# ctxnn/GenConViT

Hardware: AMD Instinct MI355X
Metric: frames/sec (224x224, ed+vae forward) (higher is better)
Workload: dtype f16

## Files before the change

### genconvit_amd/_lib.py

```python
from __future__ import annotations

import ctypes
import ctypes.util
import json
import os
import threading

_HERE = os.path.dirname(os.path.abspath(__file__))
LIB_PATH = os.environ.get("GCV_LIB_PATH") or os.path.join(_HERE, "lib", "libgenconvit_hip.so")

GCV_F32, GCV_BF16, GCV_F16 = 0, 1, 2
ACT_NONE, ACT_RELU, ACT_GELU, ACT_LEAKY = 0, 1, 2, 3
A_PLAIN, A_IM2COL3_POOL, A_IM2COL3_S2 = 0, 1, 2
EPI_BIAS_ACT, EPI_RESID, EPI_POOL4, EPI_CONVT, EPI_SPLITK = 0, 1, 2, 3, 4

c_void_p, c_int, c_int64, c_float, c_char_p, c_size_t = (ctypes.c_void_p, ctypes.c_int, ctypes.c_int64,
                                                         ctypes.c_float, ctypes.c_char_p, ctypes.c_size_t)


class TensorDesc(ctypes.Structure):
    _fields_ = [("name", c_char_p), ("data", c_void_p), ("numel", c_int64), ("on_device", c_int)]


class GemmArgs(ctypes.Structure):
# ... 7 lines not shown
    "gcv_last_error": (c_char_p, []),
    "gcv_create": (c_int, [ctypes.POINTER(c_void_p), c_int, c_int, c_int]),
    "gcv_create_arch": (c_int, [ctypes.POINTER(c_void_p), c_int, c_int, c_int, c_int]),
    "gcv_handle_arch": (c_int, [c_void_p]),
    "gcv_destroy": (None, [c_void_p]),
    "gcv_workspace_bytes": (c_size_t, [c_void_p]),
    "gcv_load_ed": (c_int, [c_void_p, ctypes.POINTER(TensorDesc), c_int]),
    "gcv_load_vae": (c_int, [c_void_p, ctypes.POINTER(TensorDesc), c_int]),
    "gcv_load_swin": (c_int, [c_void_p, ctypes.POINTER(TensorDesc), c_int, c_char_p]),
    "gcv_ed_forward": (c_int, [c_void_p, c_void_p, c_int, c_void_p, c_void_p]),
    "gcv_vae_forward": (c_int, [c_void_p, c_void_p, c_void_p, c_int, c_void_p, c_void_p, c_void_p, c_void_p, c_void_p]),
    "gcv_genconvit_forward": (c_int, [c_void_p, c_void_p, c_void_p, c_void_p, c_int, c_void_p, c_void_p]),
    "gcv_ed_explain": (c_int, [c_void_p, c_void_p, c_int, c_void_p, c_void_p, c_void_p, c_void_p, c_void_p]),
    "gcv_vae_explain": (c_int, [c_void_p, c_void_p, c_void_p, c_int, c_void_p, c_void_p, c_void_p, c_void_p, c_void_p]),
    "gcv_genconvit_explain": (c_int, [c_void_p, c_void_p, c_void_p, c_void_p, c_int, c_void_p, c_void_p, c_void_p,
                                      c_void_p, c_void_p]),
    "gcv_ed_explain_at": (c_int, [c_void_p, c_void_p, c_int, c_void_p, c_int, c_void_p, c_void_p, c_void_p, c_void_p]),
    "gcv_vae_explain_at": (c_int, [c_void_p, c_void_p, c_void_p, c_int, c_void_p, c_int, c_void_p, c_void_p, c_void_p,
                                   c_void_p]),
    "gcv_genconvit_explain_at": (c_int, [c_void_p, c_void_p, c_void_p, c_void_p, c_int, c_void_p, c_int, c_void_p, c_void_p,
                                         c_void_p, c_void_p]),
    "gcv_comm_available": (c_int, []),
    "gcv_comm_count": (c_int, [c_void_p]),
    "gcv_comm_unique_id": (c_int, [c_void_p]),
    "gcv_comm_create": (c_int, [ctypes.POINTER(c_void_p), c_int, c_int, c_void_p, c_int]),
    "gcv_comm_destroy": (None, [c_void_p]),
    "gcv_allgather_logits": (c_int, [c_void_p, c_void_p, c_int, c_void_p, c_void_p]),
    "gcv_convnext_forward": (c_int, [c_void_p, c_int, c_void_p, c_int, c_int, c_void_p, c_void_p]),
    "gcv_swin_forward": (c_int, [c_void_p, c_void_p, c_int, c_void_p, c_void_p]),
    "gcv_vote": (c_int, [c_void_p, c_int, c_void_p, c_void_p]),
    "gcv_preprocess": (c_int, [c_int, c_void_p, c_void_p, c_int, c_int, c_int, c_void_p]),
    "gcv_face_crop_resize": (c_int, [c_void_p, c_int, c_int, c_int, c_void_p, c_int, c_void_p, c_int, c_void_p]),
    "gcv_face_crop_preprocess": (c_int, [c_int, c_void_p, c_int, c_int, c_int, c_void_p, c_int, c_void_p, c_int, c_void_p]),
    "gcv_cam_overlay": (c_int, [c_void_p, c_int, c_int, c_int, c_void_p, c_int, c_void_p, c_int, c_int, c_void_p, c_float,
                                c_int, c_void_p, c_void_p]),
    "gcv_track_match": (c_int, [c_void_p, c_int, c_int, c_int, c_void_p, c_int, c_int, c_int, c_void_p, c_void_p]),
    "gcv_track_chain": (c_int, [c_void_p, c_int, c_int, c_int, c_void_p, c_int, c_int, c_int, c_int, c_void_p, c_void_p]),
    "gcv_frame_hist": (c_int, [c_void_p, c_int, c_int, c_int, c_int, c_void_p, c_void_p]),
    "gcv_hist_diff": (c_int, [c_void_p, c_int, c_int, c_void_p, c_void_p]),
    "gcv_frame_cells": (c_int, [c_void_p, c_int, c_int, c_int, c_int, c_void_p, c_void_p]),
    "gcv_blend_fit": (c_int, [c_void_p, c_int, c_int, c_int, c_void_p, c_void_p]),
    "gcv_hist_diff_lag": (c_int, [c_void_p, c_int, c_int, c_int, c_void_p, c_void_p]),
    "gcv_face_quality": (c_int, [c_void_p, c_int, c_int, c_int, c_void_p, c_int, c_int, c_void_p, c_void_p]),
    "gcv_face_signature": (c_int, [c_void_p, c_int, c_int, c_int, c_void_p, c_int, c_void_p, c_void_p]),
    "gcv_sig_link": (c_int, [c_void_p, c_void_p, c_int, c_int, c_void_p, c_void_p]),
    "gcv_vote_segments": (c_int, [c_void_p, c_int, c_int, c_void_p, c_int, c_void_p, c_void_p]),
    "gcv_vote_windows": (c_int, [c_void_p, c_int, c_int, c_void_p, c_int, c_void_p, c_void_p, c_void_p]),
    "gcv_tap_set": (c_int, [c_void_p, c_char_p, c_void_p, c_size_t]),
    "gcv_tap_clear": (c_int, [c_void_p]),
    "gcv_tap_written": (c_int, [c_void_p, c_char_p]),
    "gcv_profile_enable": (c_int, [c_void_p, c_int]),
    "gcv_profile_report": (c_char_p, [c_void_p]),
    "gcv_k_gemm": (c_int, [c_int, c_int, c_int, ctypes.POINTER(GemmArgs), c_void_p]),
    "gcv_k_stem_ln": (c_int, [c_int, c_void_p, c_int64, c_int64, c_int64, c_int64, c_void_p, c_void_p, c_void_p,
                              c_void_p, c_void_p, c_int, c_int, c_int, c_float, c_void_p]),
    "gcv_k_stem_ln_c": (c_int, [c_int, c_void_p, c_int64, c_int64, c_int64, c_int64, c_void_p, c_void_p, c_void_p,
                                c_void_p, c_void_p, c_int, c_int, c_int, c_int, c_float, c_void_p]),
    "gcv_k_dwconv7_ln": (c_int, [c_int, c_void_p, c_void_p, c_void_p, c_void_p, c_void_p, c_void_p, c_int, c_int,
                                 c_int, c_int, c_float, c_void_p]),
    "gcv_dw_plan": (c_int, [c_int, c_int, c_int, c_int, c_int, c_int, c_void_p]),
    "gcv_convnext_res_ok": (c_int, [c_int, c_int]),
    "gcv_k_ln_patchify": (c_int, [c_int, c_void_p, c_void_p, c_void_p, c_void_p, c_int, c_int, c_int, c_int, c_float,
                                  c_void_p]),
    "gcv_k_layernorm_rows": (c_int, [c_int, c_void_p, c_void_p, c_void_p, c_void_p, c_int64, c_int, c_float, c_void_p]),
    "gcv_k_pool_ln": (c_int, [c_int, c_void_p, c_void_p, c_void_p, c_void_p, c_int, c_int, c_int, c_float, c_void_p]),
    "gcv_k_pool_ln_rows": (c_int, [c_int, c_void_p, c_void_p, c_void_p, c_void_p, c_int, c_int, c_int, c_float, c_int, c_int,
                                   c_int, c_void_p]),
    "gcv_k_conv3_first": (c_int, [c_int, c_void_p, c_int64, c_int64, c_int64, c_int64, c_void_p, c_void_p, c_void_p,
                                  c_int, c_int, c_int, c_int, c_int, c_void_p]),
    "gcv_k_convt2_small": (c_int, [c_int, c_void_p, c_void_p, c_void_p, c_void_p, c_int, c_int, c_int, c_int, c_void_p]),
    "gcv_k_reparam": (c_int, [c_int, c_void_p, c_int, c_void_p, c_void_p, c_void_p, c_void_p, c_int, c_int, c_void_p]),
    "gcv_k_head_tail": (c_int, [c_int, c_void_p, c_void_p, c_void_p, c_void_p, c_int, c_int, c_void_p]),
    "gcv_k_head_tail_splitk": (c_int, [c_int, c_void_p, c_int, c_void_p, c_int, c_void_p, c_void_p, c_void_p, c_int, c_int,
                                       c_void_p]),
    "gcv_k_resize_mse": (c_int, [c_int, c_void_p, c_void_p, c_void_p, c_void_p, c_void_p, c_int, c_void_p]),
    "gcv_k_swin_window_attn": (c_int, [c_int, c_void_p, c_void_p, c_void_p, c_int, c_int, c_int, c_int, c_int, c_int,
                                       c_void_p]),
    "gcv_k_patch_merge_ln": (c_int, [c_int, c_void_p, c_void_p, c_void_p, c_void_p, c_int, c_int, c_int, c_int, c_float,
                                     c_void_p]),
    "gcv_k_mean_tokens": (c_int, [c_int, c_void_p, c_void_p, c_int, c_int, c_int, c_void_p]),
    "gcv_k_head_bwd": (c_int, [c_int, c_void_p, c_int, c_void_p, c_void_p, c_void_p, c_void_p, c_void_p, c_void_p, c_void_p,
                               c_int, c_int, c_void_p]),
    "gcv_k_bb_bwd": (c_int, [c_int, c_void_p, c_void_p, c_void_p, c_int, c_int, c_void_p]),
    "gcv_k_cam": (c_int, [c_int, c_int, c_int, c_void_p, c_void_p, c_int, c_int, c_int, c_int, c_int, c_int, c_void_p,
                          c_void_p, c_void_p, c_void_p, c_float, c_int, c_void_p]),
    "gcv_k_pool_ln_bwd": (c_int, [c_int, c_int, c_int, c_void_p, c_void_p, c_int, c_int, c_int, c_int, c_void_p, c_void_p,
                                  c_void_p, c_float, c_int, c_void_p]),
    "gcv_k_scale_rows": (c_int, [c_int, c_void_p, c_void_p, c_void_p, c_void_p, c_int, c_int, c_void_p]),
    "gcv_k_gelu_bwd": (c_int, [c_int, c_void_p, c_void_p, c_void_p, c_void_p, c_int, c_int, c_void_p]),
    "gcv_k_dw_ln_bwd": (c_int, [c_int, c_void_p, c_void_p, c_void_p, c_void_p, c_void_p, c_void_p, c_void_p, c_int, c_int,
                                c_int, c_float, c_void_p]),
    "gcv_k_dw_dgrad_res": (c_int, [c_void_p, c_void_p, c_void_p, c_int, c_int, c_int, c_void_p]),
    "gcv_k_down_ln_bwd": (c_int, [c_int, c_void_p, c_void_p, c_void_p, c_void_p, c_void_p, c_int, c_int, c_int, c_float,
                                  c_void_p]),
    "gcv_k_cam2": (c_int, [c_int, c_int, c_int, c_void_p, c_void_p, c_void_p, c_void_p, c_int, c_int, c_int, c_int, c_int,
                           c_int, c_void_p, c_void_p, c_void_p, c_int, c_void_p]),
    "gcv_k_fused_mlp": (c_int, [c_int, c_int, c_void_p, c_void_p, c_void_p, c_void_p, c_void_p, c_void_p, c_void_p,
                                c_void_p, c_int, c_void_p]),
    "gcv_k_fused_mlp_lnp": (c_int, [c_int, c_int, c_void_p, c_void_p, c_void_p, c_void_p, c_void_p, c_void_p, c_void_p,
                                    c_void_p, c_void_p, c_float, c_int, c_void_p, c_void_p, c_void_p, c_void_p, c_void_p,
                                    c_int, c_void_p]),
    "gcv_k_fused_mlp_timed": (c_int, [c_int, c_int, c_void_p, c_void_p, c_void_p, c_void_p, c_void_p, c_void_p,
                                      c_void_p, c_void_p, c_int, c_int, c_void_p, c_void_p]),
}

_lib = None
# ... 791 lines not shown
```

### genconvit_amd/csrc/api.hip

```cpp
#include "../../include/genconvit_hip.h"

#include <dlfcn.h>

#include <cstdio>
#include <cstdlib>
#include <cstring>
#include <map>
#include <mutex>
#include <set>
#include <sstream>
#include <vector>

#include "cam.h"
#include "cam_bwd.h"
#include "cnx_mlp.h"
#include "gemm.h"
#include "kernels.h"
#include "net.h"

namespace gcv {
static thread_local std::string g_err;
void set_error(const std::string& msg) { g_err = msg; }
const char* get_error() { return g_err.c_str(); }

int ensure_dynamic_lds(const void* fn, int bytes) {
  static std::mutex mu;
  static std::map<std::pair<const void*, int>, int> done;
  int dev = 0;
  GCV_CHECK_HIP(hipGetDevice(&dev));
  std::lock_guard<std::mutex> lk(mu);
  auto it = done.find({fn, dev});
  if (it != done.end() && it->second >= bytes) return 0;
  GCV_CHECK_HIP(hipFuncSetAttribute(fn, hipFuncAttributeMaxDynamicSharedMemorySize, bytes));
  done[{fn, dev}] = bytes;
  return 0;
}

hipEvent_t Profiler::get_event() {
  if (next_event == pool.size()) {
    hipEvent_t e;
    if (hipEventCreate(&e) != hipSuccess) return nullptr;
    pool.push_back(e);
  }
  return pool[next_event++];
}
Profiler::~Profiler() {
  for (hipEvent_t e : pool) (void)hipEventDestroy(e);
}

namespace {
struct Roctx {
  int (*push)(const char*) = nullptr;
  int (*pop)() = nullptr;
  Roctx() {
    for (const char* lib : {"librocprofiler-sdk-roctx.so", "librocprofiler-sdk-roctx.so.1", "libroctx64.so", "libroctx64.so.4"}) {
      void* h = dlopen(lib, RTLD_NOW | RTLD_GLOBAL);
      if (!h) continue;
      push = reinterpret_cast<int (*)(const char*)>(dlsym(h, "roctxRangePushA"));
      pop = reinterpret_cast<int (*)()>(dlsym(h, "roctxRangePop"));
      if (push && pop) return;
      push = nullptr; pop = nullptr;
    }
  }
};
Roctx& roctx() { static Roctx r; return r; }
}
bool tap_name_known(const std::string& name, int arch) {
  auto make = [](int arch) {
    std::set<std::string> n;
// ... 471 lines not shown
int gcv_tap_written(gcv_handle* h, const char* name) {
  GCV_REQUIRE(h && name, "null handle / tap name");
  auto it = h->net->taps.find(name);
  GCV_REQUIRE(it != h->net->taps.end(), std::string("no tap '") + name + "' is set");
  return it->second.need != 0 && it->second.mask == it->second.need ? 1 : 0;
}

size_t gcv_workspace_bytes(const gcv_handle* h) { return h ? h->net->workspace_bytes() : 0; }

int gcv_handle_arch(const gcv_handle* h) { return h ? h->net->arch : -1; }

int gcv_profile_enable(gcv_handle* h, int on) {
  GCV_REQUIRE(h, "null handle");
  h->net->prof.enabled = on != 0;
  h->net->prof.reset();
  return 0;
}

const char* gcv_profile_report(gcv_handle* h) {
  if (!h) return "[]";
  Profiler& p = h->net->prof;
  struct Agg { int n = 0; double ms = 0, flops = 0, bytes = 0; };
  std::map<std::string, Agg> agg;
  std::vector<std::string> order;
  for (auto& r : p.recs) {
    float ms = 0.0f;
    if (hipEventSynchronize(r.e1) != hipSuccess || hipEventElapsedTime(&ms, r.e0, r.e1) != hipSuccess) ms = -1.0f;
    if (!agg.count(r.tag)) order.push_back(r.tag);
    Agg& a = agg[r.tag];
    a.n += 1; a.ms += ms; a.flops += r.flops; a.bytes += r.bytes;
  }
  std::ostringstream os;
  os.precision(9);
  os << "[";
  for (size_t i = 0; i < order.size(); ++i) {
    const Agg& a = agg[order[i]];
    os << (i ? "," : "") << "{\"tag\":\"" << order[i] << "\",\"launches\":" << a.n << ",\"ms\":" << a.ms
       << ",\"flops\":" << a.flops << ",\"bytes\":" << a.bytes << "}";
  }
  os << "]";
  h->report = os.str();
  p.reset();
  return h->report.c_str();
}

#define DISPATCH_DT(dt, CALL)                                    \
  switch (dt) {                                                  \
    case GCV_F32:  { typedef float T;  return CALL; }            \
    case GCV_BF16: { typedef bf16_t T; return CALL; }            \
    case GCV_F16:  { typedef half_t T; return CALL; }            \
    default: set_error("bad dtype"); return -2;                  \
  }

int gcv_k_gemm(int dtype, int a_mode, int epi, const gcv_gemm_args* a, gcv_stream stream) {
  GCV_REQUIRE(a, "null args");
  GemmArgs g{};
  g.A = a->A; g.Wt = a->Wt; g.C = a->C; g.bias = a->bias; g.gamma = a->gamma; g.resid = a->resid;
  g.partial = a->partial; g.M = a->M; g.N = a->N; g.K = a->K; g.lda = a->lda; g.ldc = a->ldc; g.act = a->act;
  g.splitk = a->splitk; g.k_per_split = a->k_per_split; g.H = a->H; g.W = a->W; g.cin_log2 = a->cin_log2;
  g.cout_log2 = a->cout_log2;
  DISPATCH_DT(dtype, launch_gemm<T>(g, a_mode, epi, (hipStream_t)stream));
}

int gcv_k_stem_ln(int dtype, const void* x, int64_t sb, int64_t sc, int64_t sy, int64_t sx, const float* wp,
                  const float* bias, const float* lnw, const float* lnb, void* out, int nimg, int Ho, int Wo,
                  float eps, gcv_stream s) {
  DISPATCH_DT(dtype, launch_stem_ln<T>((const T*)x, sb, sc, sy, sx, wp, bias, lnw, lnb, (T*)out, nimg, Ho, Wo, eps,
                                       (hipStream_t)s));
}

int gcv_k_stem_ln_c(int dtype, const void* x, int64_t sb, int64_t sc, int64_t sy, int64_t sx, const float* wp,
                    const float* bias, const float* lnw, const float* lnb, void* out, int nimg, int Ho, int Wo, int C,
                    float eps, gcv_stream s) {
  DISPATCH_DT(dtype, launch_stem_ln<T>((const T*)x, sb, sc, sy, sx, wp, bias, lnw, lnb, (T*)out, nimg, Ho, Wo, eps,
                                       (hipStream_t)s, C));
}

int gcv_k_dwconv7_ln(int dtype, const void* x, const float* wdw, const float* bdw, const float* lnw,
                     const float* lnb, void* y, int nimg, int H, int W, int C, float eps, gcv_stream s) {
  DISPATCH_DT(dtype, launch_dwconv7_ln<T>((const T*)x, wdw, bdw, lnw, lnb, (T*)y, nimg, H, W, C, eps, (hipStream_t)s));
}

int gcv_dw_plan(int dtype, int nimg, int H, int W, int C, int aligned, int* out5) {
  GCV_REQUIRE(out5, "null out5");
  DwPlan p;
  auto put = [&](int rc) {
    if (rc == 0) { out5[0] = (int)p.kind; out5[1] = p.grid; out5[2] = p.block; out5[3] = p.lds; out5[4] = p.band_rows; }
    return rc;
  };
  DISPATCH_DT(dtype, put(dw_plan<T>(p, nimg, H, W, C, aligned != 0)));
}

int gcv_convnext_res_ok(int arch, int res) { return cnx_res_ok(arch, res) ? 1 : 0; }

int gcv_k_ln_patchify(int dtype, const void* x, const float* w, const float* b, void* out, int nimg, int H, int W,
                      int C, float eps, gcv_stream s) {
  DISPATCH_DT(dtype, launch_ln_patchify<T>((const T*)x, w, b, (T*)out, nimg, H, W, C, eps, (hipStream_t)s));
}

int gcv_k_layernorm_rows(int dtype, const void* x, const float* w, const float* b, void* out, int64_t rows, int C,
                         float eps, gcv_stream s) {
  DISPATCH_DT(dtype, launch_layernorm_rows<T>((const T*)x, w, b, (T*)out, rows, C, eps, (hipStream_t)s));
}

int gcv_k_pool_ln(int dtype, const void* x, const float* w, const float* b, void* out, int nimg, int HW, int C,
                  float eps, gcv_stream s) {
  DISPATCH_DT(dtype, launch_pool_ln<T>((const T*)x, w, b, (T*)out, nimg, HW, C, eps, (hipStream_t)s));
}

int gcv_k_pool_ln_rows(int dtype, const void* x, const float* w, const float* b, void* out, int nimg, int HW, int C,
                       float eps, int seg_n, int row_stride, int row0, gcv_stream s) {
  DISPATCH_DT(dtype, launch_pool_ln<T>((const T*)x, w, b, (T*)out, nimg, HW, C, eps, (hipStream_t)s, seg_n, row_stride,
                                       row0));
}
// ... 223 lines not shown
```

### genconvit_amd/csrc/gemm.h

```cpp
#pragma once
#include <type_traits>

#include "common.h"

namespace gcv {

enum { A_PLAIN = 0, A_IM2COL3_POOL = 1, A_IM2COL3_S2 = 2 };
enum { EPI_BIAS_ACT = 0, EPI_RESID = 1, EPI_POOL4 = 2, EPI_CONVT = 3, EPI_SPLITK = 4 };

struct GemmArgs {
  const void* A;
  const void* Wt;
  void* C;
  const float* bias;
  const float* gamma;
  const void* resid;
  float* partial;
  int M, N, K;
  int lda, ldc;
  int act;
  int splitk;
  int k_per_split;
  int H, W;
  int cin_log2;
// ... 498 lines not shown
    if (idx >= ROWS * PPR) break;
    const int rl = idx / PPR, pc = idx - rl * PPR;
    const int n = n0 + 4 * pc;
    const int m = m0 + ((EPI == EPI_POOL4) ? 4 * rl : rl);
    if (m >= g.M || n >= g.N) continue;
    f32x4 v;
    if (EPI == EPI_POOL4) {
#pragma unroll
      for (int k = 0; k < 4; ++k) {
        f32x4 w;
        if (STAGE_F32) {
          w = *(const f32x4*)(sC + (4 * rl + k) * SROW + 4 * pc);
        } else {
          const t4 h = *(const t4*)(sC + (4 * rl + k) * SROW + 2 * pc);
          w = f32x4{to_f(h[0]), to_f(h[1]), to_f(h[2]), to_f(h[3])};
        }
        if (k == 0) v = w;
        else
#pragma unroll
          for (int e = 0; e < 4; ++e) v[e] = fmaxf(v[e], w[e]);
      }
    } else if (STAGE_F32) {
      v = *(const f32x4*)(sC + rl * SROW + 4 * pc);
    }
    int64_t o;
    if (EPI == EPI_CONVT) {
      const int xx = m % g.W, tt = m / g.W;
      const int yy = tt % g.H, bb = tt / g.H;
      const int dq = n >> g.cout_log2, co = n & ((1 << g.cout_log2) - 1);
      o = ((((int64_t)bb * 2 * g.H + 2 * yy + (dq >> 1)) * 2 * g.W + 2 * xx + (dq & 1)) << g.cout_log2) + co;
    } else if (EPI == EPI_POOL4) {
      o = (int64_t)(m >> 2) * g.ldc + n;
    } else {
      o = (int64_t)m * g.ldc + n;
    }
    if (EPI == EPI_SPLITK) {
      *(f32x4*)(g.partial + ((int64_t)blockIdx.y * g.M + m) * g.N + n) = v;
      continue;
    }
    if (EPI == EPI_RESID) {
#pragma unroll
      for (int e = 0; e < 4; ++e) v[e] += to_f(rres[it][e]);
    }
    if (STAGE_F32 || EPI == EPI_POOL4) {
      t4 out = {from_f<T>(v[0]), from_f<T>(v[1]), from_f<T>(v[2]), from_f<T>(v[3])};
      *(t4*)(Cp + o) = out;
    } else {
      *(t4*)(Cp + o) = *(const t4*)(sC + rl * SROW + 2 * pc);
    }
  }
}

template <typename T> int launch_gemm(const GemmArgs& g, int a_mode, int epi, hipStream_t stream);
const char* gemm_family_name(int a_mode, int epi);

}
```

### genconvit_amd/csrc/gemm_bf16.hip

```cpp
#include "gemm_impl.h"
namespace gcv { template int launch_gemm<bf16_t>(const GemmArgs&, int, int, hipStream_t); }
```

### genconvit_amd/csrc/gemm_f16.hip

```cpp
#include "gemm_impl.h"
namespace gcv { template int launch_gemm<half_t>(const GemmArgs&, int, int, hipStream_t); }

GCV_GLDS_STAMP_READER
```

### genconvit_amd/csrc/gemm_f32.hip

```cpp
#include "gemm_impl.h"
namespace gcv { template int launch_gemm<float>(const GemmArgs&, int, int, hipStream_t); }
```

### genconvit_amd/csrc/gemm_impl.h

```cpp
#pragma once
#include "gemm.h"
#include "conv_direct.h"
#include "gemm_glds_impl.h"

namespace gcv {

template <typename T, int BM, int BN, int WM, int WN, int BKB, int AMODE, int EPI, int ACT>
static int launch_cfg(const GemmArgs& g, hipStream_t s) {
  constexpr int SMEM = GemmSmem<T, BM, BN, BKB, EPI>::bytes;
  if (SMEM > 64 * 1024) GCV_ENSURE_LDS((gemm_kernel<T, BM, BN, WM, WN, BKB, AMODE, EPI, ACT>), SMEM);
  const int ntm = cdiv(g.M, BM), ntn = cdiv(g.N, BN);
  dim3 grid(ntm * ntn, EPI == EPI_SPLITK ? g.splitk : 1, 1);
  hipLaunchKernelGGL((gemm_kernel<T, BM, BN, WM, WN, BKB, AMODE, EPI, ACT>), grid, dim3(256), SMEM, s, g);
  GCV_CHECK_HIP(hipGetLastError());
  return 0;
}

static inline bool aligned16(const void* p) { return (reinterpret_cast<uintptr_t>(p) & 15u) == 0; }

template <typename T> struct DefBKB { static constexpr int v = sizeof(T) == 4 ? 64 : 128; };

#define GCV_ACT_SWITCH(CALL)                                     \
  switch (g.act) {                                               \
    case ACT_NONE:  return CALL(ACT_NONE);                       \
    case ACT_RELU:  return CALL(ACT_RELU);                       \
    case ACT_GELU:  return CALL(ACT_GELU);                       \
    case ACT_LEAKY: return CALL(ACT_LEAKY);                      \
    default: set_error("bad activation code"); return -2;        \
  }

#ifndef GCV_IM2COL_SHORTK
#define GCV_IM2COL_SHORTK 1
#endif
template <typename T> int launch_gemm(const GemmArgs& g, int a_mode, int epi, hipStream_t s) {
  constexpr int EPC = DT<T>::EPC;
  constexpr int B = DefBKB<T>::v;
  constexpr int BK = B / 16 * EPC;
  GCV_REQUIRE(g.M > 0 && g.N > 0 && g.K > 0, "empty GEMM");
  GCV_REQUIRE(g.K % EPC == 0, "K must be a multiple of the 16-byte chunk");
  GCV_REQUIRE(g.N % 4 == 0, "N must be a multiple of 4");
  GCV_REQUIRE(aligned16(g.A) && aligned16(g.Wt), "A/Wt must be 16-byte aligned");
  if (epi != EPI_SPLITK) {
    GCV_REQUIRE(g.C && (reinterpret_cast<uintptr_t>(g.C) % (4 * sizeof(T))) == 0, "C must be aligned to 4 elements");
    GCV_REQUIRE(epi == EPI_CONVT || (g.ldc % 4 == 0 && g.ldc >= g.N), "ldc must be a multiple of 4 and >= N");
    GCV_REQUIRE(!g.bias || aligned16(g.bias), "bias must be 16-byte aligned");
  }
  if (a_mode == A_PLAIN) {
    GCV_REQUIRE(g.lda % EPC == 0 && g.lda >= g.K, "lda must be a chunk multiple >= K");
  } else {
    GCV_REQUIRE((1 << g.cin_log2) % EPC == 0 && g.K == 9 * (1 << g.cin_log2), "im2col: K = 9*Cin, Cin chunk-aligned");
    GCV_REQUIRE((g.H % 2) == 0 && (g.W % 2) == 0, "im2col modes need even H, W");
  }
  if (epi == EPI_SPLITK) {
    GCV_REQUIRE(g.splitk >= 1 && g.k_per_split % BK == 0 && (int64_t)g.k_per_split * g.splitk >= g.K && g.partial &&
                aligned16(g.partial), "bad split-K plan");
  }
  if (epi == EPI_RESID) GCV_REQUIRE(g.gamma && g.resid && aligned16(g.gamma), "EPI_RESID needs gamma and resid");
  if (epi == EPI_POOL4) GCV_REQUIRE(g.M % 4 == 0, "EPI_POOL4 needs M % 4 == 0");
  if (epi == EPI_CONVT) GCV_REQUIRE(g.N == 4 << g.cout_log2 && g.cout_log2 >= 2 && g.M % (g.H * g.W) == 0, "EPI_CONVT shape");
  if constexpr (sizeof(T) == 2) {
    if (gemm_glds_applicable<T>(g, a_mode, epi)) return launch_gemm_glds<T>(g, epi, s);
  }
  const bool short_k = sizeof(T) == 2 && (g.K % 64) != 0 && (g.K % 64) <= 32;

  if (a_mode == A_PLAIN && epi == EPI_BIAS_ACT) {
#define C1(A) launch_cfg<T, 32, 128, 32, 32, B, A_PLAIN, EPI_BIAS_ACT, A>(g, s)
#define C2(A) launch_cfg<T, 64, 128, 32, 64, B, A_PLAIN, EPI_BIAS_ACT, A>(g, s)
#define C3(A) launch_cfg<T, 128, 96, 32, 96, B, A_PLAIN, EPI_BIAS_ACT, A>(g, s)
#define C3S(A) launch_cfg<T, 128, 96, 32, 96, 64, A_PLAIN, EPI_BIAS_ACT, A>(g, s)
#define C4(A) launch_cfg<T, 128, 128, 64, 64, B, A_PLAIN, EPI_BIAS_ACT, A>(g, s)
    const int t128 = cdiv(g.M, 128) * cdiv(g.N, 128);
    if (g.M <= 32 || t128 < 48) { GCV_ACT_SWITCH(C1) }
    if (g.M <= 64 || t128 < 96) { GCV_ACT_SWITCH(C2) }
    if (g.N % 96 == 0) {
      if (short_k) { GCV_ACT_SWITCH(C3S) }
      GCV_ACT_SWITCH(C3)
    }
    GCV_ACT_SWITCH(C4)
#undef C1
#undef C2
#undef C3
#undef C3S
#undef C4
  }
  if (a_mode == A_PLAIN && epi == EPI_RESID) {
    GCV_REQUIRE(g.act == ACT_NONE, "EPI_RESID has no activation");
    if (g.N % 96 == 0) return launch_cfg<T, 128, 96, 32, 96, B, A_PLAIN, EPI_RESID, ACT_NONE>(g, s);
    return launch_cfg<T, 128, 128, 64, 64, B, A_PLAIN, EPI_RESID, ACT_NONE>(g, s);
  }
  if (a_mode == A_PLAIN && epi == EPI_CONVT) {
    GCV_REQUIRE(g.act == ACT_RELU || g.act == ACT_LEAKY, "EPI_CONVT is built for ReLU / LeakyReLU");
    if (g.N <= 64) {
      if (short_k) {
        if (g.act == ACT_RELU) return launch_cfg<T, 128, 64, 32, 64, 64, A_PLAIN, EPI_CONVT, ACT_RELU>(g, s);
        return launch_cfg<T, 128, 64, 32, 64, 64, A_PLAIN, EPI_CONVT, ACT_LEAKY>(g, s);
      }
      if (g.act == ACT_RELU) return launch_cfg<T, 128, 64, 32, 64, B, A_PLAIN, EPI_CONVT, ACT_RELU>(g, s);
      return launch_cfg<T, 128, 64, 32, 64, B, A_PLAIN, EPI_CONVT, ACT_LEAKY>(g, s);
    }
    if (g.act == ACT_RELU) return launch_cfg<T, 128, 128, 64, 64, B, A_PLAIN, EPI_CONVT, ACT_RELU>(g, s);
    return launch_cfg<T, 128, 128, 64, 64, B, A_PLAIN, EPI_CONVT, ACT_LEAKY>(g, s);
  }
  if (a_mode == A_PLAIN && epi == EPI_SPLITK) {
    if (g.M <= 32) return launch_cfg<T, 32, 128, 32, 32, B, A_PLAIN, EPI_SPLITK, ACT_NONE>(g, s);
    if (g.M <= 64) return launch_cfg<T, 64, 128, 32, 64, B, A_PLAIN, EPI_SPLITK, ACT_NONE>(g, s);
    return launch_cfg<T, 128, 128, 64, 64, B, A_PLAIN, EPI_SPLITK, ACT_NONE>(g, s);
  }
  if (a_mode == A_IM2COL3_POOL && epi == EPI_POOL4) {
    GCV_REQUIRE(g.act == ACT_RELU, "conv3x3+pool is built for ReLU");
    if (conv_direct_applicable<T>(g, a_mode, epi)) return launch_conv_direct<T>(g, a_mode, s);
    if (short_k && GCV_IM2COL_SHORTK) {
      if (g.N <= 32) return launch_cfg<T, 128, 32, 32, 32, 64, A_IM2COL3_POOL, EPI_POOL4, ACT_RELU>(g, s);
      if (g.N <= 64) return launch_cfg<T, 128, 64, 32, 64, 64, A_IM2COL3_POOL, EPI_POOL4, ACT_RELU>(g, s);
    }
    if (g.N <= 32) return launch_cfg<T, 128, 32, 32, 32, B, A_IM2COL3_POOL, EPI_POOL4, ACT_RELU>(g, s);
    if (g.N <= 64) return launch_cfg<T, 128, 64, 32, 64, B, A_IM2COL3_POOL, EPI_POOL4, ACT_RELU>(g, s);
    return launch_cfg<T, 128, 128, 64, 64, B, A_IM2COL3_POOL, EPI_POOL4, ACT_RELU>(g, s);
  }
  if (a_mode == A_IM2COL3_S2 && epi == EPI_BIAS_ACT) {
    GCV_REQUIRE(g.act == ACT_LEAKY, "conv3x3 stride 2 is built for LeakyReLU");
    if (conv_direct_applicable<T>(g, a_mode, epi)) return launch_conv_direct<T>(g, a_mode, s);
    if (short_k && GCV_IM2COL_SHORTK) {
      if (g.N <= 32) return launch_cfg<T, 128, 32, 32, 32, 64, A_IM2COL3_S2, EPI_BIAS_ACT, ACT_LEAKY>(g, s);
      if (g.N <= 64) return launch_cfg<T, 128, 64, 32, 64, 64, A_IM2COL3_S2, EPI_BIAS_ACT, ACT_LEAKY>(g, s);
    }
    if (g.N <= 32) return launch_cfg<T, 128, 32, 32, 32, B, A_IM2COL3_S2, EPI_BIAS_ACT, ACT_LEAKY>(g, s);
    if (g.N <= 64) return launch_cfg<T, 128, 64, 32, 64, B, A_IM2COL3_S2, EPI_BIAS_ACT, ACT_LEAKY>(g, s);
    return launch_cfg<T, 128, 128, 64, 64, B, A_IM2COL3_S2, EPI_BIAS_ACT, ACT_LEAKY>(g, s);
  }
  set_error("launch_gemm: unsupported (a_mode, epilogue) combination");
  return -3;
}

}
```

### genconvit_amd/csrc/isa_report.py

```python
#!/usr/bin/env python3
import re
import subprocess
import sys


def demangle(n):
    for tool in ("/opt/rocm/lib/llvm/bin/llvm-cxxfilt", "c++filt"):
        try:
            out = subprocess.run([tool, n], capture_output=True, text=True).stdout.strip()
            if out:
                return out
        except Exception:
            pass
    return n


SCRATCH_BUDGET = [
    (r"pw2f_kernelI\w+?Li384ELi384ELi3ELi8EE", 28),
    (r"xs_mlp_kernelI\w+?Li192ELb[01]EE", 20),
    (r"dwconv7_ln_roll_kernelI\w+?Li96ELi4EE", 8),
    (r"dwconv7_ln_kernelI\w+?Li768EE", 88),
]


def kernel_meta(path):
    out = []
    s = open(path).read()
    for b in re.split(r'^\s+- \.agpr_count:', s, flags=re.M)[1:]:
        g = lambda k: int(re.search(r'\.%s:\s+(\S+)' % k, b).group(1))
        out.append((re.search(r'\.name:\s+(\S+)', b).group(1),
                    dict(agpr=int(b.split()[0]), vgpr=g('vgpr_count'), sgpr=g('sgpr_count'), spill=g('vgpr_spill_count'),
                         scratch=g('private_segment_fixed_size'), lds=g('group_segment_fixed_size'))))
    return out


def report(paths):
    for path in paths:
        for name, m in kernel_meta(path):
            nm = re.sub(r'\(.*', '', demangle(name))[:110]
            print(f"{nm:110s} vgpr {m['vgpr']:>4} agpr {m['agpr']:>4} sgpr {m['sgpr']:>4} spill {m['spill']:>3} "
                  f"scratch {m['scratch']:>4} lds {m['lds']}")


def check_scratch(path):
    findings = []
    for name, m in kernel_meta(path):
        nm = re.sub(r'\(.*', '', demangle(name))
        budget = next((b for pat, b in SCRATCH_BUDGET if re.search(pat, name)), 0)
        if m['scratch'] > budget:
            findings.append(f"{path}: {nm[:100]}: {m['scratch']} bytes of scratch per lane ({m['spill']} spilled VGPRs), budget "
                            f"{budget} — register cliff (isa_report.py check 3)")
    return findings


REG = re.compile(r'\b([va])(\d+)\b|\b([va])\[(\d+):(\d+)\]')


def regs_of(operand):
    out = set()
    for m in REG.finditer(operand):
        if m.group(1):
            out.add((m.group(1), int(m.group(2))))
        else:
            out.update((m.group(3), i) for i in range(int(m.group(4)), int(m.group(5)) + 1))
    return out


def split_ops(rest):
    return [o.strip() for o in rest.split(',')] if rest else []

# ... 116 lines not shown
```

### include/genconvit_hip.h

```cpp
#ifndef GENCONVIT_HIP_H
#define GENCONVIT_HIP_H

#include <stddef.h>
#include <stdint.h>

#ifdef __cplusplus
extern "C" {
#endif

#if defined(GCV_BUILD)
#pragma GCC visibility push(default)
#endif

typedef struct gcv_handle gcv_handle;
typedef void* gcv_stream;

enum { GCV_F32 = 0, GCV_BF16 = 1, GCV_F16 = 2 };
enum { GCV_CONVNEXT_TINY = 0, GCV_CONVNEXT_LARGE = 1 };
enum { GCV_LARGE_MAX_BATCH = 256 };
enum { GCV_ACT_NONE = 0, GCV_ACT_RELU = 1, GCV_ACT_GELU = 2, GCV_ACT_LEAKY = 3 };

typedef struct {
  const char* name;
  const void* data;
// ... 58 lines not shown

int gcv_track_chain(const void* frames_u8_nhwc, int nframes, int H, int W, const int* jobs11, int n, int max_steps, int grid,
                    int radius, int* out4, gcv_stream s);

int gcv_frame_hist(const void* frames_u8_nhwc, int nframes, int H, int W, int regions, uint32_t* hist_u32,
                   gcv_stream stream);
int gcv_hist_diff(const uint32_t* hist_u32, int nframes, int regions, uint32_t* dist_u32, gcv_stream stream);

int gcv_frame_cells(const void* frames_u8_nhwc, int nframes, int H, int W, int grid, uint32_t* cells_u32,
                    gcv_stream stream);
int gcv_blend_fit(const uint32_t* cells_u32, int nframes, int grid, int lag, int64_t* fit_i64, gcv_stream stream);
int gcv_hist_diff_lag(const uint32_t* hist_u32, int nframes, int regions, int lag, uint32_t* dist_u32, gcv_stream stream);

int gcv_face_quality(const void* frames_u8_nhwc, int nframes, int H, int W, const int* boxes5, int n, int grid,
                     int64_t* out8, gcv_stream stream);

int gcv_face_signature(const void* frames_u8_nhwc, int nframes, int H, int W, const int* boxes5, int n, void* sig384,
                       gcv_stream stream);
int gcv_sig_link(const void* sig384, const int* owner, int n, int tracks, uint32_t* out_u32, gcv_stream stream);

int gcv_vote(const float* logits, int rows, float* mean2, gcv_stream stream);

int gcv_vote_segments(const float* logits, int batch, int nets, const int* offsets, int n_videos, float* mean2,
                      gcv_stream stream);

int gcv_vote_windows(const float* logits, int batch, int nets, const int* ranges2, int n_ranges, float* frame_p,
                     float* mean2, gcv_stream stream);

typedef struct gcv_comm gcv_comm;
int  gcv_comm_available(void);
int  gcv_comm_count(gcv_comm* c);
int  gcv_comm_unique_id(void* id128);
int  gcv_comm_create(gcv_comm** c, int world, int rank, const void* id128, int device);
void gcv_comm_destroy(gcv_comm* c);
int  gcv_allgather_logits(gcv_comm* c, const float* local, int n_local, float* all, gcv_stream stream);

int gcv_profile_enable(gcv_handle* h, int on);
const char* gcv_profile_report(gcv_handle* h);

int gcv_tap_set(gcv_handle* h, const char* name, void* dst, size_t bytes);
int gcv_tap_clear(gcv_handle* h);
int gcv_tap_written(gcv_handle* h, const char* name);

enum { GCV_A_PLAIN = 0, GCV_A_IM2COL3_POOL = 1, GCV_A_IM2COL3_S2 = 2 };
enum { GCV_EPI_BIAS_ACT = 0, GCV_EPI_RESID = 1, GCV_EPI_POOL4 = 2, GCV_EPI_CONVT = 3, GCV_EPI_SPLITK = 4 };

typedef struct {
  const void* A; const void* Wt; void* C;
  const float* bias; const float* gamma; const void* resid; float* partial;
  int M, N, K, lda, ldc, act, splitk, k_per_split, H, W, cin_log2, cout_log2;
} gcv_gemm_args;

int gcv_k_gemm(int dtype, int a_mode, int epi, const gcv_gemm_args* a, gcv_stream s);
int gcv_k_stem_ln(int dtype, const void* x, int64_t sb, int64_t sc, int64_t sy, int64_t sx, const float* wp,
                  const float* bias, const float* lnw, const float* lnb, void* out, int nimg, int Ho, int Wo,
                  float eps, gcv_stream s);
int gcv_k_stem_ln_c(int dtype, const void* x, int64_t sb, int64_t sc, int64_t sy, int64_t sx, const float* wp,
                    const float* bias, const float* lnw, const float* lnb, void* out, int nimg, int Ho, int Wo, int C,
                    float eps, gcv_stream s);
int gcv_k_dwconv7_ln(int dtype, const void* x, const float* wdw, const float* bdw, const float* lnw,
                     const float* lnb, void* y, int nimg, int H, int W, int C, float eps, gcv_stream s);
int gcv_dw_plan(int dtype, int nimg, int H, int W, int C, int aligned, int* out5);
int gcv_convnext_res_ok(int arch, int res);
int gcv_k_ln_patchify(int dtype, const void* x, const float* w, const float* b, void* out, int nimg, int H, int W,
                      int C, float eps, gcv_stream s);
int gcv_k_layernorm_rows(int dtype, const void* x, const float* w, const float* b, void* out, int64_t rows, int C,
                         float eps, gcv_stream s);
int gcv_k_pool_ln(int dtype, const void* x, const float* w, const float* b, void* out, int nimg, int HW, int C,
                  float eps, gcv_stream s);
int gcv_k_pool_ln_rows(int dtype, const void* x, const float* w, const float* b, void* out, int nimg, int HW, int C,
                       float eps, int seg_n, int row_stride, int row0, gcv_stream s);
int gcv_k_conv3_first(int dtype, const void* x, int64_t sb, int64_t sc, int64_t sy, int64_t sx, const float* wp,
                      const float* bias, void* out, int nimg, int H, int W, int pool, int act, gcv_stream s);
int gcv_k_convt2_small(int dtype, const void* x, const float* wp, const float* bias, void* out, int nimg, int H,
                       int W, int act, gcv_stream s);
int gcv_k_reparam(int dtype, const float* partial, int splitk, const float* bias, const float* eps, float* mu_out,
                  void* z_nhwc, int B, int N, gcv_stream s);
int gcv_k_head_tail(int dtype, const void* h, const float* w, const float* bias, float* logits, int B, int K,
                    gcv_stream s);
int gcv_k_head_tail_splitk(int dtype, const float* partial, int splitk, const float* b1, int act, const float* w,
                           const float* bias, float* logits, int B, int K, gcv_stream s);
int gcv_k_resize_mse(int dtype, const void* xhat, const void* img, void* recon, float* msepart, float* mse, int B,
                     gcv_stream s);

int gcv_k_swin_window_attn(int dtype, const void* qkv, const float* rpb, void* out, int nimg, int H, int W, int C,
                           int nH, int shift, gcv_stream s);
int gcv_k_patch_merge_ln(int dtype, const void* x, const float* w, const float* b, void* out, int nimg, int H, int W,
                         int C, float eps, gcv_stream s);
int gcv_k_mean_tokens(int dtype, const void* x, void* out, int nimg, int L, int C, gcv_stream s);

int gcv_k_head_bwd(int dtype, const float* partial, int S, const float* b1, const float* fc2_w, const float* logits,
                   const int* target, const void* fc_w, const void* bb_pre, float* dfeat, int B, int act, gcv_stream s);
int gcv_k_bb_bwd(int dtype, const float* dfeat, const void* w, float* dpool, int rows, int C, gcv_stream s);
int gcv_k_cam(int dtype, int C, int npass, const void* A0, const void* A1, int side0, int side1, int off0, int off1,
              int cam_ld, int up_pass, const float* lnw, const float* dpool, float* cam, float* cam224, float eps, int B,
              gcv_stream s);
int gcv_k_pool_ln_bwd(int dtype, int C, int npass, const void* A0, const void* A1, int hw0, int hw1, int tok0_0,
                      int tok0_1, const float* lnw, const float* dpool, float* dA, float eps, int B, gcv_stream s);
int gcv_k_scale_rows(int dtype, const float* g, const float* gamma, void* out, float* inv, int M, int C, gcv_stream s);
int gcv_k_gelu_bwd(int dtype, const float* dh, const float* inv_in, void* pre, float* inv_out, int M, int C4,
                   gcv_stream s);
int gcv_k_dw_ln_bwd(int dtype, const void* x, const float* dw_w, const float* dw_b, const float* ln_w, const float* dxln,
                    const float* inv, float* ddw, int nimg, int side, int C, float eps, gcv_stream s);
int gcv_k_dw_dgrad_res(const float* ddw, const float* dw_w, float* g, int nimg, int side, int C, gcv_stream s);
int gcv_k_down_ln_bwd(int dtype, const void* x, const float* ln_w, const float* dP, const float* inv, float* dA2,
                      int nimg, int side2, int C2, float eps, gcv_stream s);
// ... 23 lines not shown
```

Measured before the change: 18830.

## Add weight-streaming split-K GEMM kernel for mid-size-M 16-bit GEMMs

Adds a split-K GEMM kernel for 16-bit inputs with 64<M<=128. Each wave streams whole 32-column weight strips straight into registers through an 8-deep ring of loads, while the small A tile is double-buffered in swizzled LDS. Work is spread across about 256 workgroups so that the weight stream, probably the large VAE linear layer, runs at HBM bandwidth. A planning query API and a microbenchmark are added alongside. The risk is high register pressure and a heuristic grid sized for a fixed CU count.

```diff
diff --git a/genconvit_amd/_lib.py b/genconvit_amd/_lib.py
--- a/genconvit_amd/_lib.py
+++ b/genconvit_amd/_lib.py
@@ -83,6 +83,8 @@
     "gcv_profile_enable": (c_int, [c_void_p, c_int]),
     "gcv_profile_report": (c_char_p, [c_void_p]),
     "gcv_k_gemm": (c_int, [c_int, c_int, c_int, ctypes.POINTER(GemmArgs), c_void_p]),
+    "gcv_gemm_plan": (c_int, [c_int, c_int, c_int, ctypes.POINTER(GemmArgs), c_void_p]),
+    "gcv_gemm_stream_item": (c_int, [c_int, c_int, c_int, c_void_p]),
     "gcv_k_stem_ln": (c_int, [c_int, c_void_p, c_int64, c_int64, c_int64, c_int64, c_void_p, c_void_p, c_void_p,
                               c_void_p, c_void_p, c_int, c_int, c_int, c_float, c_void_p]),
     "gcv_k_stem_ln_c": (c_int, [c_int, c_void_p, c_int64, c_int64, c_int64, c_int64, c_void_p, c_void_p, c_void_p,
diff --git a/genconvit_amd/csrc/api.hip b/genconvit_amd/csrc/api.hip
--- a/genconvit_amd/csrc/api.hip
+++ b/genconvit_amd/csrc/api.hip
@@ -15,6 +15,7 @@
 #include "cam_bwd.h"
 #include "cnx_mlp.h"
 #include "gemm.h"
+#include "gemm_stream.h"
 #include "kernels.h"
 #include "net.h"
 
@@ -592,14 +593,38 @@
     default: set_error("bad dtype"); return -2;                  \
   }
 
-int gcv_k_gemm(int dtype, int a_mode, int epi, const gcv_gemm_args* a, gcv_stream stream) {
-  GCV_REQUIRE(a, "null args");
+static GemmArgs gemm_args_of(const gcv_gemm_args* a) {
   GemmArgs g{};
   g.A = a->A; g.Wt = a->Wt; g.C = a->C; g.bias = a->bias; g.gamma = a->gamma; g.resid = a->resid;
   g.partial = a->partial; g.M = a->M; g.N = a->N; g.K = a->K; g.lda = a->lda; g.ldc = a->ldc; g.act = a->act;
   g.splitk = a->splitk; g.k_per_split = a->k_per_split; g.H = a->H; g.W = a->W; g.cin_log2 = a->cin_log2;
   g.cout_log2 = a->cout_log2;
+  return g;
+}
+
+int gcv_k_gemm(int dtype, int a_mode, int epi, const gcv_gemm_args* a, gcv_stream stream) {
+  GCV_REQUIRE(a, "null args");
+  const GemmArgs g = gemm_args_of(a);
   DISPATCH_DT(dtype, launch_gemm<T>(g, a_mode, epi, (hipStream_t)stream));
+}
+
+int gcv_gemm_plan(int dtype, int a_mode, int epi, const gcv_gemm_args* a, int* out4) {
+  GCV_REQUIRE(a && out4, "null args");
+  const GemmArgs g = gemm_args_of(a);
+  GemmPlan p;
+  auto put = [&](int rc) {
+    if (rc == 0) { out4[0] = (int)p.kind; out4[1] = p.grid; out4[2] = p.block; out4[3] = p.groups; }
+    return rc;
+  };
+  DISPATCH_DT(dtype, put(gemm_plan<T>(p, g, a_mode, epi)));
+}
+
+int gcv_gemm_stream_item(int N, int splitk, int bid, int* out3) {
+  GCV_REQUIRE(out3 && N >= 32 && N % 32 == 0 && splitk >= 1, "N a positive multiple of 32, splitk >= 1");
+  const int groups = gemm_stream_groups(N / 32, splitk);
+  GCV_REQUIRE(bid >= 0 && bid < splitk * groups, "workgroup index outside the grid");
+  gemm_stream_item(bid, splitk, N / 32, groups, out3[0], out3[1], out3[2]);
+  return 0;
 }
 
 int gcv_k_stem_ln(int dtype, const void* x, int64_t sb, int64_t sc, int64_t sy, int64_t sx, const float* wp,
diff --git a/genconvit_amd/csrc/gemm.h b/genconvit_amd/csrc/gemm.h
--- a/genconvit_amd/csrc/gemm.h
+++ b/genconvit_amd/csrc/gemm.h
@@ -574,6 +574,9 @@
 }
 
 template <typename T> int launch_gemm(const GemmArgs& g, int a_mode, int epi, hipStream_t stream);
+enum class GemmKind { Tile, Glds, ConvDirect, Stream };
+struct GemmPlan { GemmKind kind; int grid, block, groups; };
+template <typename T> int gemm_plan(GemmPlan& p, const GemmArgs& g, int a_mode, int epi);
 const char* gemm_family_name(int a_mode, int epi);
 
 }
diff --git a/genconvit_amd/csrc/gemm_bf16.hip b/genconvit_amd/csrc/gemm_bf16.hip
--- a/genconvit_amd/csrc/gemm_bf16.hip
+++ b/genconvit_amd/csrc/gemm_bf16.hip
@@ -1,2 +1,5 @@
 #include "gemm_impl.h"
-namespace gcv { template int launch_gemm<bf16_t>(const GemmArgs&, int, int, hipStream_t); }
+namespace gcv {
+template int launch_gemm<bf16_t>(const GemmArgs&, int, int, hipStream_t);
+template int gemm_plan<bf16_t>(GemmPlan&, const GemmArgs&, int, int);
+}
diff --git a/genconvit_amd/csrc/gemm_f16.hip b/genconvit_amd/csrc/gemm_f16.hip
--- a/genconvit_amd/csrc/gemm_f16.hip
+++ b/genconvit_amd/csrc/gemm_f16.hip
@@ -1,4 +1,7 @@
 #include "gemm_impl.h"
-namespace gcv { template int launch_gemm<half_t>(const GemmArgs&, int, int, hipStream_t); }
+namespace gcv {
+template int launch_gemm<half_t>(const GemmArgs&, int, int, hipStream_t);
+template int gemm_plan<half_t>(GemmPlan&, const GemmArgs&, int, int);
+}
 
 GCV_GLDS_STAMP_READER
diff --git a/genconvit_amd/csrc/gemm_f32.hip b/genconvit_amd/csrc/gemm_f32.hip
--- a/genconvit_amd/csrc/gemm_f32.hip
+++ b/genconvit_amd/csrc/gemm_f32.hip
@@ -1,2 +1,5 @@
 #include "gemm_impl.h"
-namespace gcv { template int launch_gemm<float>(const GemmArgs&, int, int, hipStream_t); }
+namespace gcv {
+template int launch_gemm<float>(const GemmArgs&, int, int, hipStream_t);
+template int gemm_plan<float>(GemmPlan&, const GemmArgs&, int, int);
+}
diff --git a/genconvit_amd/csrc/gemm_impl.h b/genconvit_amd/csrc/gemm_impl.h
--- a/genconvit_amd/csrc/gemm_impl.h
+++ b/genconvit_amd/csrc/gemm_impl.h
@@ -1,6 +1,7 @@
 #pragma once
 #include "gemm.h"
 #include "conv_direct.h"
+#include "gemm_stream.h"
 #include "gemm_glds_impl.h"
 
 namespace gcv {
@@ -32,10 +33,9 @@
 #ifndef GCV_IM2COL_SHORTK
 #define GCV_IM2COL_SHORTK 1
 #endif
-template <typename T> int launch_gemm(const GemmArgs& g, int a_mode, int epi, hipStream_t s) {
+template <typename T> static int gemm_validate(const GemmArgs& g, int a_mode, int epi) {
   constexpr int EPC = DT<T>::EPC;
-  constexpr int B = DefBKB<T>::v;
-  constexpr int BK = B / 16 * EPC;
+  constexpr int BK = DefBKB<T>::v / 16 * EPC;
   GCV_REQUIRE(g.M > 0 && g.N > 0 && g.K > 0, "empty GEMM");
   GCV_REQUIRE(g.K % EPC == 0, "K must be a multiple of the 16-byte chunk");
   GCV_REQUIRE(g.N % 4 == 0, "N must be a multiple of 4");
@@ -58,6 +58,27 @@
   if (epi == EPI_RESID) GCV_REQUIRE(g.gamma && g.resid && aligned16(g.gamma), "EPI_RESID needs gamma and resid");
   if (epi == EPI_POOL4) GCV_REQUIRE(g.M % 4 == 0, "EPI_POOL4 needs M % 4 == 0");
   if (epi == EPI_CONVT) GCV_REQUIRE(g.N == 4 << g.cout_log2 && g.cout_log2 >= 2 && g.M % (g.H * g.W) == 0, "EPI_CONVT shape");
+  return 0;
+}
+
+template <typename T> int gemm_plan(GemmPlan& p, const GemmArgs& g, int a_mode, int epi) {
+  GCV_TRY(gemm_validate<T>(g, a_mode, epi));
+  p = GemmPlan{GemmKind::Tile, 0, 256, 0};
+  if constexpr (sizeof(T) == 2) {
+    if (gemm_glds_applicable<T>(g, a_mode, epi)) {
+      p = GemmPlan{GemmKind::Glds, cdiv(g.M, kGldsBM) * (g.N / kGldsBN), 256, 0};
+    } else if (gemm_stream_applicable<T>(g, a_mode, epi)) {
+      p = GemmPlan{GemmKind::Stream, gemm_stream_grid(g), kGsThreads, gemm_stream_groups(g.N / 32, g.splitk)};
+    } else if (conv_direct_applicable<T>(g, a_mode, epi)) {
+      p = GemmPlan{GemmKind::ConvDirect, conv_direct_grid(g.M, g.N), 256, 0};
+    }
+  }
+  return 0;
+}
+
+template <typename T> int launch_gemm(const GemmArgs& g, int a_mode, int epi, hipStream_t s) {
+  constexpr int B = DefBKB<T>::v;
+  GCV_TRY(gemm_validate<T>(g, a_mode, epi));
   if constexpr (sizeof(T) == 2) {
     if (gemm_glds_applicable<T>(g, a_mode, epi)) return launch_gemm_glds<T>(g, epi, s);
   }
@@ -102,6 +123,7 @@
     return launch_cfg<T, 128, 128, 64, 64, B, A_PLAIN, EPI_CONVT, ACT_LEAKY>(g, s);
   }
   if (a_mode == A_PLAIN && epi == EPI_SPLITK) {
+    if (gemm_stream_applicable<T>(g, a_mode, epi)) return launch_gemm_stream<T>(g, s);
     if (g.M <= 32) return launch_cfg<T, 32, 128, 32, 32, B, A_PLAIN, EPI_SPLITK, ACT_NONE>(g, s);
     if (g.M <= 64) return launch_cfg<T, 64, 128, 32, 64, B, A_PLAIN, EPI_SPLITK, ACT_NONE>(g, s);
     return launch_cfg<T, 128, 128, 64, 64, B, A_PLAIN, EPI_SPLITK, ACT_NONE>(g, s);
diff --git a/genconvit_amd/csrc/gemm_stream.h b/genconvit_amd/csrc/gemm_stream.h
--- /dev/null
+++ b/genconvit_amd/csrc/gemm_stream.h
@@ -0,0 +1,192 @@
+#pragma once
+#include <algorithm>
+#include <type_traits>
+
+#include "gemm.h"
+
+namespace gcv {
+
+constexpr int kGsThreads = 512;
+constexpr int kGsWaves = 8;
+constexpr int kGsBlocksPerWave = 2;
+constexpr int kGsMaxBlocks = kGsWaves * kGsBlocksPerWave;
+constexpr int kGsBK = 64;
+constexpr int kGsRows = 128;
+constexpr int kGsTileBytes = kGsRows * kGsBK * 2;
+constexpr int kGsRing = 8;
+constexpr int kGsCUs = 256;
+
+#ifndef GCV_GEMM_STREAM
+#define GCV_GEMM_STREAM 1
+#endif
+#ifndef GCV_GEMM_STREAM_NT
+#define GCV_GEMM_STREAM_NT 0
+#endif
+
+__host__ __device__ inline int gemm_stream_groups(int ncb, int splitk) {
+  const int want = kGsCUs / splitk > 1 ? kGsCUs / splitk : 1;
+  const int need = (ncb + kGsMaxBlocks - 1) / kGsMaxBlocks;
+  const int g = need > want ? need : want;
+  return g < ncb ? g : ncb;
+}
+__host__ __device__ inline void gemm_stream_item(int bid, int splitk, int ncb, int groups, int& split, int& cb0, int& ncol) {
+  split = bid % splitk;
+  const int grp = bid / splitk;
+  const int base = ncb / groups, rem = ncb % groups;
+  cb0 = grp * base + (grp < rem ? grp : rem);
+  ncol = base + (grp < rem ? 1 : 0);
+}
+
+template <typename T, int NJ>
+__device__ __forceinline__ void gemm_stream_wave(const GemmArgs& g, unsigned char* smem, int split, int cb, int tid) {
+  constexpr int RING = kGsRing;
+  static_assert(RING == 8, "the K loop below names two K tiles' ring slots per trip");
+  constexpr int NJA = NJ > 0 ? NJ : 1;
+  const int lane = tid & 63;
+  const int lr = lane & 31, lh = lane >> 5;
+  const int kbeg = split * g.k_per_split;
+  const int nkt = g.k_per_split / kGsBK;
+  const int nks = nkt * 4;
+
+  const T* wp[NJA];
+#pragma unroll
+  for (int j = 0; j < NJ; ++j) wp[j] = (const T*)g.Wt + (size_t)((cb + kGsWaves * j) * 32 + lr) * g.K + kbeg + 8 * lh;
+  auto load_w = [&](int j, int s) {
+    const T* p = wp[j] + 16 * (s < nks ? s : 0);
+#if GCV_GEMM_STREAM_NT
+    return __builtin_nontemporal_load((const u32x4*)p);
+#else
+    return *(const u32x4*)p;
+#endif
+  };
+
+  const T* ap[2];
+  int a_dst[2];
+#pragma unroll
+  for (int s = 0; s < 2; ++s) {
+    const int idx = tid + s * kGsThreads;
+    const int row = idx >> 3, c = idx & 7;
+    ap[s] = (const T*)g.A + (size_t)min(row, g.M - 1) * g.lda + kbeg + 8 * c;
+    a_dst[s] = row * 128 + ((c ^ ((row >> 1) & 7)) << 4);
+  }
+  u32x4 areg[2];
+  auto fetch_a = [&](int kt) {
+    const int k = min(kt, nkt - 1) * kGsBK;
+#pragma unroll
+    for (int s = 0; s < 2; ++s) areg[s] = *(const u32x4*)(ap[s] + k);
+  };
+  auto stage_a = [&](int buf) {
+#pragma unroll
+    for (int s = 0; s < 2; ++s) *(u32x4*)(smem + buf * kGsTileBytes + a_dst[s]) = areg[s];
+  };
+
+  f32x16 acc[4][NJA];
+#pragma unroll
+  for (int i = 0; i < 4; ++i)
+#pragma unroll
+    for (int j = 0; j < NJA; ++j)
+#pragma unroll
+      for (int r = 0; r < 16; ++r) acc[i][j][r] = 0.0f;
+
+  fetch_a(0);
+  u32x4 wf[NJA][RING];
+#pragma unroll
+  for (int s = 0; s < RING; ++s) {
+#pragma unroll
+    for (int j = 0; j < NJ; ++j) wf[j][s] = load_w(j, s);
+    __builtin_amdgcn_sched_barrier(0);
+  }
+  stage_a(0);
+  __syncthreads();
+
+  const int a_row = lr * 128, a_sw = (lr >> 1) & 7;
+
+  auto tile = [&](int kt, auto U) {
+    constexpr int u = decltype(U)::value;
+    fetch_a(kt + 1);
+    __builtin_amdgcn_sched_barrier(0);
+    if constexpr (NJ > 0) {
+      const unsigned char* sA = smem + (kt & 1) * kGsTileBytes + a_row;
+      u32x4 af[2][4];
+      auto read_a = [&](int t) {
+#pragma unroll
+        for (int i = 0; i < 4; ++i) af[t & 1][i] = *(const u32x4*)(sA + i * (32 * 128) + (((2 * t + lh) ^ a_sw) << 4));
+      };
+      read_a(0);
+#pragma unroll
+      for (int t = 0; t < 4; ++t) {
+        if (t + 1 < 4) read_a(t + 1);
+#pragma unroll
+        for (int j = 0; j < NJ; ++j) {
+#pragma unroll
+          for (int i = 0; i < 4; ++i) Mfma<T>::run(wf[j][4 * u + t], af[t & 1][i], acc[i][j]);
+          wf[j][4 * u + t] = load_w(j, 4 * kt + t + RING);
+          __builtin_amdgcn_sched_barrier(0);
+        }
+      }
+    }
+    stage_a((kt + 1) & 1);
+    __syncthreads();
+  };
+  int kt = 0;
+  for (; kt + 1 < nkt; kt += 2) {
+    tile(kt, std::integral_constant<int, 0>{});
+    tile(kt + 1, std::integral_constant<int, 1>{});
+  }
+  if (kt < nkt) tile(kt, std::integral_constant<int, 0>{});
+
+#pragma unroll
+  for (int j = 0; j < NJ; ++j) {
+    const int n0 = (cb + kGsWaves * j) * 32 + 4 * lh;
+#pragma unroll
+    for (int i = 0; i < 4; ++i) {
+      const int m = 32 * i + lr;
+      if (m < g.M) {
+        float* o = g.partial + ((size_t)split * g.M + m) * g.N + n0;
+#pragma unroll
+        for (int q = 0; q < 4; ++q)
+          *(f32x4*)(o + 8 * q) = (f32x4){acc[i][j][4 * q], acc[i][j][4 * q + 1], acc[i][j][4 * q + 2], acc[i][j][4 * q + 3]};
+      }
+    }
+  }
+}
+
+template <typename T>
+__global__ void __launch_bounds__(kGsThreads) gemm_stream_kernel(const GemmArgs g, const int groups) {
+  static_assert(sizeof(T) == 2, "16-bit storage");
+  __shared__ __attribute__((aligned(16))) unsigned char smem[2 * kGsTileBytes];
+  const int tid = threadIdx.x;
+  const int wave = __builtin_amdgcn_readfirstlane(tid >> 6);
+  int split, cb0, ncol;
+  gemm_stream_item(blockIdx.x, g.splitk, g.N >> 5, groups, split, cb0, ncol);
+  if (wave + kGsWaves < ncol) gemm_stream_wave<T, 2>(g, smem, split, cb0 + wave, tid);
+  else if (wave < ncol) gemm_stream_wave<T, 1>(g, smem, split, cb0 + wave, tid);
+  else gemm_stream_wave<T, 0>(g, smem, split, cb0, tid);
+}
+
+static inline bool gs_aligned16(const void* p) { return (reinterpret_cast<uintptr_t>(p) & 15u) == 0; }
+
+template <typename T> static bool gemm_stream_applicable(const GemmArgs& g, int a_mode, int epi) {
+  if (!GCV_GEMM_STREAM || sizeof(T) != 2) return false;
+  if (a_mode != A_PLAIN || epi != EPI_SPLITK || g.act != ACT_NONE) return false;
+  if (g.M <= 64 || g.M > kGsRows) return false;
+  if (g.lda != g.K || g.N % 32 != 0 || g.splitk < 1) return false;
+  if (g.k_per_split <= 0 || g.k_per_split % kGsBK != 0 || (int64_t)g.splitk * g.k_per_split != g.K) return false;
+  if ((int64_t)g.splitk * gemm_stream_groups(g.N / 32, g.splitk) > 0x7fffffff) return false;
+  return gs_aligned16(g.A) && gs_aligned16(g.Wt) && g.partial && gs_aligned16(g.partial);
+}
+
+static inline int gemm_stream_grid(const GemmArgs& g) { return g.splitk * gemm_stream_groups(g.N / 32, g.splitk); }
+
+template <typename T> static int launch_gemm_stream(const GemmArgs& g, hipStream_t s) {
+  if constexpr (sizeof(T) == 2) {
+    const int groups = gemm_stream_groups(g.N / 32, g.splitk);
+    hipLaunchKernelGGL((gemm_stream_kernel<T>), dim3(g.splitk * groups), dim3(kGsThreads), 0, s, g, groups);
+    GCV_CHECK_HIP(hipGetLastError());
+    return 0;
+  }
+  set_error("launch_gemm_stream: 16-bit storage only");
+  return -3;
+}
+
+}
diff --git a/genconvit_amd/csrc/isa_report.py b/genconvit_amd/csrc/isa_report.py
--- a/genconvit_amd/csrc/isa_report.py
+++ b/genconvit_amd/csrc/isa_report.py
@@ -16,6 +16,7 @@
 
 
 SCRATCH_BUDGET = [
+    (r"gemm_stream_kernelI", 0),
     (r"pw2f_kernelI\w+?Li384ELi384ELi3ELi8EE", 28),
     (r"xs_mlp_kernelI\w+?Li192ELb[01]EE", 20),
     (r"dwconv7_ln_roll_kernelI\w+?Li96ELi4EE", 8),
diff --git a/include/genconvit_hip.h b/include/genconvit_hip.h
--- a/include/genconvit_hip.h
+++ b/include/genconvit_hip.h
@@ -134,6 +134,8 @@
 } gcv_gemm_args;
 
 int gcv_k_gemm(int dtype, int a_mode, int epi, const gcv_gemm_args* a, gcv_stream s);
+int gcv_gemm_plan(int dtype, int a_mode, int epi, const gcv_gemm_args* a, int* out4);
+int gcv_gemm_stream_item(int N, int splitk, int bid, int* out3);
 int gcv_k_stem_ln(int dtype, const void* x, int64_t sb, int64_t sc, int64_t sy, int64_t sx, const float* wp,
                   const float* bias, const float* lnw, const float* lnb, void* out, int nimg, int Ho, int Wo,
                   float eps, gcv_stream s);
diff --git a/profiles/mu_gemm_stream_kernel.py b/profiles/mu_gemm_stream_kernel.py
--- /dev/null
+++ b/profiles/mu_gemm_stream_kernel.py
@@ -0,0 +1,48 @@
+#!/usr/bin/env python3
+import ctypes, math, os, sys
+import torch
+ROOT = os.path.dirname(os.path.dirname(os.path.abspath(__file__)))
+sys.path.insert(0, ROOT)
+from genconvit_amd import _lib
+
+M = int(sys.argv[1]) if len(sys.argv) > 1 else 128
+dt = {"f16": torch.float16, "bf16": torch.bfloat16}[sys.argv[2] if len(sys.argv) > 2 else "f16"]
+iters = int(sys.argv[3]) if len(sys.argv) > 3 else 20
+N, K, S = 12544, 25088, 8
+dev = torch.device("cuda", 0)
+lib = _lib.load()
+torch.manual_seed(0)
+A = (torch.rand(M, K, device=dev) * 2 - 1).to(dt)
+W = ((torch.rand(N, K, device=dev) * 2 - 1) / math.sqrt(K)).to(dt)
+part = torch.zeros(S, M, N, device=dev)
+flush = torch.empty(512 << 20, dtype=torch.uint8, device=dev)
+g = _lib.GemmArgs(A.data_ptr(), W.data_ptr(), None, None, None, None, part.data_ptr(), M, N, K, K, 0, 0, S, K // S, 0, 0, 0, 0)
+plan = (ctypes.c_int * 4)()
+kind = "?"
+if hasattr(lib, "gcv_gemm_plan") and lib.gcv_gemm_plan(_lib.dtype_code(dt), _lib.A_PLAIN, _lib.EPI_SPLITK, ctypes.byref(g), plan) == 0:
+    kind = ["tile", "glds", "conv_direct", "stream"][plan[0]]
+fn = lambda: _lib.check(lib.gcv_k_gemm(_lib.dtype_code(dt), _lib.A_PLAIN, _lib.EPI_SPLITK, ctypes.byref(g),
+                                       _lib.current_stream_ptr(dev)), "gemm")
+for _ in range(3):
+    fn()
+torch.cuda.synchronize()
+cold = []
+for i in range(iters):
+    flush.fill_(i & 1)
+    e0, e1 = torch.cuda.Event(enable_timing=True), torch.cuda.Event(enable_timing=True)
+    e0.record(); fn(); e1.record()
+    torch.cuda.synchronize()
+    cold.append(e0.elapsed_time(e1) * 1e3)
+e0, e1 = torch.cuda.Event(enable_timing=True), torch.cuda.Event(enable_timing=True)
+e0.record()
+for _ in range(iters):
+    fn()
+e1.record()
+torch.cuda.synchronize()
+replay = e0.elapsed_time(e1) * 1e3 / iters
+cold.sort()
+wbytes = N * K * 2
+print(f"mu gemm M={M} {sys.argv[2] if len(sys.argv) > 2 else 'f16'} lib={os.path.basename(_lib.LIB_PATH)} kernel={kind}: "
+      f"cold median {cold[len(cold) // 2]:.1f} us (min {cold[0]:.1f}, max {cold[-1]:.1f}) = "
+      f"{wbytes / cold[len(cold) // 2] / 1e6:.2f} TB/s of weights;  replay {replay:.1f} us = {wbytes / replay / 1e6:.2f} TB/s   "
+      f"checksum {part.double().sum().item():.6e}")
```

Result: no change. 18710 (-0.6%).
